# alexandre01/deepsvg

Measured on AMD Instinct MI355X. Metric: SVG icons/sec (train step) hierarchical_ordered d=256, higher is better.
Workload: dtype bf16; 1 GPU; hierarchical_ordered (Hierarchical, use_vae=False) G=8 S=30 d_model=256 ff=512 H=8 L=4x4; full train step = forward + SVGLoss + backward + grad-clip 1.0 + AdamW; dropout 0.1; global_batch=512, batch_per_gpu=512, parallelism=dp1, hip_graph=True, encoder_layout=packed (valid tokens only, exact)

## Files before the change

deepsvg_amd/csrc/dsvg_common.h:

```cpp
#pragma once
#include <hip/hip_runtime.h>
#include <stdint.h>
#include <string.h>
#include <stdio.h>

#define DSVG_F32 0
#define DSVG_BF16 1

typedef uint16_t bf16_t;

extern "C" const char* dsvg_last_error(void);
void dsvg_set_error(const char* fmt, ...);

#define DSVG_CHECK_ARG(cond, ...)                \
    do {                                         \
        if (!(cond)) {                           \
            dsvg_set_error(__VA_ARGS__);         \
            return -1;                           \
        }                                        \
    } while (0)

#define DSVG_LAUNCH_CHECK(name)                                                        \
    do {                                                                               \
        hipError_t _e = hipGetLastError();                                             \
        if (_e != hipSuccess) {                                                        \
            dsvg_set_error("%s: launch failed: %s", name, hipGetErrorString(_e));      \
            return -2;                                                                 \
        }                                                                              \
    } while (0)

#define DSVG_ENSURE_LDS(kern, bytes)                                                                      \
    do {                                                                                                  \
        static size_t _dsvg_cap = 64 * 1024;                                                              \
        if ((size_t)(bytes) > _dsvg_cap) {                                                                \
            (void)hipFuncSetAttribute((const void*)(kern), hipFuncAttributeMaxDynamicSharedMemorySize,    \
                                      (int)(bytes));                                                      \
            _dsvg_cap = (size_t)(bytes);                                                                  \
        }                                                                                                 \
    } while (0)

__device__ __forceinline__ float bf2f(bf16_t h) { return __uint_as_float(((uint32_t)h) << 16); }
typedef __bf16 dsvg_bf2 __attribute__((ext_vector_type(2)));
typedef float dsvg_f2 __attribute__((ext_vector_type(2)));
__device__ __forceinline__ bf16_t f2bf(float f) {
    const __bf16 b = (__bf16)f;
    return __builtin_bit_cast(bf16_t, b);
}
__device__ __forceinline__ uint32_t f2bf_pk(float lo, float hi) {
    const dsvg_f2 v = {lo, hi};
    const dsvg_bf2 b = __builtin_convertvector(v, dsvg_bf2);
    return __builtin_bit_cast(uint32_t, b);
}

template <typename T> struct Elem;
template <> struct Elem<float> {
    typedef float4 raw4;
    static __device__ __forceinline__ float ld(const float* p) { return *p; }
    static __device__ __forceinline__ void st(float* p, float v) { *p = v; }
    static __device__ __forceinline__ void ld4(const float* p, float (&v)[4]) {
        float4 t = *reinterpret_cast<const float4*>(p);
        v[0] = t.x; v[1] = t.y; v[2] = t.z; v[3] = t.w;
    }
    static __device__ __forceinline__ void st4(float* p, const float (&v)[4]) {
        *reinterpret_cast<float4*>(p) = make_float4(v[0], v[1], v[2], v[3]);
    }
};
template <> struct Elem<bf16_t> {
    typedef uint2 raw4;
    static __device__ __forceinline__ float ld(const bf16_t* p) { return bf2f(*p); }
    static __device__ __forceinline__ void st(bf16_t* p, float v) { *p = f2bf(v); }
    static __device__ __forceinline__ void ld4(const bf16_t* p, float (&v)[4]) {
        uint2 t = *reinterpret_cast<const uint2*>(p);
        v[0] = __uint_as_float(t.x << 16); v[1] = __uint_as_float(t.x & 0xffff0000u);
        v[2] = __uint_as_float(t.y << 16); v[3] = __uint_as_float(t.y & 0xffff0000u);
    }
    static __device__ __forceinline__ void st4(bf16_t* p, const float (&v)[4]) {
        uint2 t;
        t.x = f2bf_pk(v[0], v[1]);
        t.y = f2bf_pk(v[2], v[3]);
        *reinterpret_cast<uint2*>(p) = t;
    }
};

__device__ __forceinline__ void row32_load(const float* p, float (&v)[32]) {
#pragma unroll
// ... 42 lines not shown
};
__device__ __forceinline__ DropCtx drop_make(float p, const uint64_t* seed_ptr, uint32_t site) {
    DropCtx c;
    c.on = (p > 0.f) && (seed_ptr != nullptr);
    if (c.on) {
        uint64_t seed = *seed_ptr;
        c.s0 = dsvg_hash32((uint32_t)seed ^ (site * 0x9e3779b1u));
        c.s1 = dsvg_hash32((uint32_t)(seed >> 32) + site * 0x85ebca77u + 0x165667b1u);
        uint32_t t = (uint32_t)(p * 65536.f + 0.5f);
        c.thresh = t > 65535u ? 65535u : t;
        c.scale = 65536.f / (float)(65536u - c.thresh);
    } else {
        c.s0 = c.s1 = 0; c.thresh = 0; c.scale = 1.f;
    }
    return c;
}
__device__ __forceinline__ uint32_t drop_group(const DropCtx& c, uint64_t g) {
    const uint32_t h = dsvg_hash32((uint32_t)g ^ c.s0);
    return (h ^ c.s1) + (uint32_t)(g >> 32) * 0x9e3779b1u;
}
__device__ __forceinline__ uint32_t drop_word(uint32_t h, uint32_t i) {
    const uint32_t c = ((0x7feb352du * (i + 1u)) ^ (0x846ca68bu >> i)) | 1u;
    return (h * c) ^ __umulhi(h, c);
}
__device__ __forceinline__ float drop_mult(const DropCtx& c, uint64_t idx) {
    if (!c.on) return 1.f;
    const uint32_t slot = (uint32_t)idx & 7u;
    const uint32_t w = drop_word(drop_group(c, idx >> 3), slot >> 1);
    const uint32_t draw = (slot & 1u) ? (w >> 16) : (w & 0xffffu);
    return draw < c.thresh ? 0.f : c.scale;
}
__device__ __forceinline__ void drop_mult8(const DropCtx& c, uint64_t idx8, float (&m)[8]) {
    if (!c.on) {
#pragma unroll
        for (int e = 0; e < 8; ++e) m[e] = 1.f;
        return;
    }
    const uint32_t h = drop_group(c, idx8 >> 3);
#pragma unroll
    for (int i = 0; i < 4; ++i) {
        const uint32_t w = drop_word(h, i);
        m[2 * i] = (w & 0xffffu) < c.thresh ? 0.f : c.scale;
        m[2 * i + 1] = (w >> 16) < c.thresh ? 0.f : c.scale;
    }
}

__device__ __forceinline__ uint32_t attn_drop_row(const DropCtx& c, uint64_t row, uint32_t key_block) {
    const uint64_t g = row * 8ull + key_block;
    const uint32_t h = dsvg_hash32((uint32_t)g ^ c.s0);
    return dsvg_hash32(h + (uint32_t)(g >> 32) * 0x9e3779b1u + c.s1);
}
__device__ __forceinline__ float attn_drop_key(const DropCtx& c, uint32_t hrow, uint32_t key) {
    if (!c.on) return 1.f;
    const uint32_t w = drop_word(hrow, (key & 31u) >> 1);
    const uint32_t draw = (key & 1u) ? (w >> 16) : (w & 0xffffu);
    return draw < c.thresh ? 0.f : c.scale;
}
__device__ __forceinline__ float attn_drop_mult(const DropCtx& c, uint64_t row, uint32_t key) {
    if (!c.on) return 1.f;
    return attn_drop_key(c, attn_drop_row(c, row, key >> 5), key);
}

__device__ __forceinline__ float dsvg_gumbel_from_word(uint32_t w) {
    const float u = ((float)(w >> 9) + 0.5f) * (1.f / 8388608.f);
    return -__logf(-__logf(u));
}
__device__ __forceinline__ float dsvg_gumbel(const DropCtx& c, uint64_t row, uint32_t k4, uint32_t col) {
    return dsvg_gumbel_from_word(drop_word(drop_group(c, row * k4 + (col >> 2)), col & 3u));
}

__device__ __forceinline__ float wave_sum(float v) {
#pragma unroll
    for (int o = 32; o > 0; o >>= 1) v += __shfl_xor(v, o, 64);
    return v;
}
__device__ __forceinline__ float wave_max(float v) {
#pragma unroll
    for (int o = 32; o > 0; o >>= 1) v = fmaxf(v, __shfl_xor(v, o, 64));
    return v;
}

static inline int dsvg_cdiv(long long a, long long b) { return (int)((a + b - 1) / b); }

__host__ __device__ inline size_t dsvg_splitk_slice(size_t M, size_t N, bool rowsums) {
    return (M * N + (rowsums ? M : 0) + 3) & ~(size_t)3;
}

int dsvg_reduce_partials_strided(const float* part, int64_t P, int64_t stride, int64_t n, float* out,
                                 int32_t accumulate, hipStream_t st);
int dsvg_reduce_partials_mixed(const float* part, int64_t P, int64_t stride, int64_t n, int64_t n_bf16, float* out,
                               int32_t accumulate, hipStream_t st);
```

deepsvg_amd/csrc/embed.hip:

```cpp
#include "dsvg_common.h"
#include "../../include/dsvg.h"

__global__ void build_masks_kernel(const float* __restrict__ commands, long long n_seq, int S, int G, int eos,
                                   uint64_t* __restrict__ key_mask, int* __restrict__ seq_visible,
                                   uint64_t* __restrict__ group_mask) {
    const long long b = (long long)blockIdx.x * blockDim.x + threadIdx.x;
    if (b >= n_seq) return;
    const float* row = commands + b * S;
    uint64_t km = 0;
    int n_eos = 0;
    bool seen = false;
    for (int s = 0; s < S; ++s) {
        const bool is_eos = ((int)row[s] == eos);
        seen |= is_eos;
        n_eos += is_eos;
        if (!seen) km |= (1ull << s);
    }
    if (key_mask) key_mask[b] = km;
    if (seq_visible) seq_visible[b] = (n_eos < S - 1) ? 1 : 0;
}
__global__ void group_mask_kernel(const int* __restrict__ seq_visible, long long n_icons, int G,
                                  uint64_t* __restrict__ group_mask) {
    const long long n = (long long)blockIdx.x * blockDim.x + threadIdx.x;
    if (n >= n_icons) return;
// ... 173 lines not shown
    hipStream_t st = (hipStream_t)stream;
    hipLaunchKernelGGL(seq_offsets_kernel, dim3(1), dim3(1024), 0, st, key_mask, (long long)n_seq, seq_off);
    DSVG_LAUNCH_CHECK("seq_offsets");
    hipLaunchKernelGGL(pack_tokens_kernel, dim3(dsvg_cdiv(n_seq * S, 256)), dim3(256), 0, st, commands, args, seq_off,
                       (long long)n_seq, S, n_args, packed_commands, packed_args, packed_pos);
    DSVG_LAUNCH_CHECK("pack_tokens");
    return 0;
}

__global__ __launch_bounds__(1024) void seq_offsets_lens_kernel(const int32_t* __restrict__ lens, long long n_seq, int S,
                                                                int32_t* __restrict__ seq_off) {
    __shared__ int part[1024];
    __shared__ int carry;
    if (threadIdx.x == 0) carry = 0;
    __syncthreads();
    for (long long base = 0; base < n_seq; base += 1024) {
        const long long b = base + threadIdx.x;
        const int len = b < n_seq ? min(max(lens[b], 0), S) : 0;
        part[threadIdx.x] = len;
        __syncthreads();
        for (int o = 1; o < 1024; o <<= 1) {
            const int v = threadIdx.x >= o ? part[threadIdx.x - o] : 0;
            __syncthreads();
            part[threadIdx.x] += v;
            __syncthreads();
        }
        if (b < n_seq) seq_off[b] = carry + part[threadIdx.x] - len;
        __syncthreads();
        if (threadIdx.x == 1023) carry += part[1023];
        __syncthreads();
    }
    if (threadIdx.x == 0) seq_off[n_seq] = carry;
}
extern "C" int dsvg_pack_tokens_lens(const float* commands, const float* args, const int32_t* lens, int64_t n_seq,
                                     int32_t S, int32_t n_args, int32_t* seq_off, float* packed_commands,
                                     float* packed_args, int32_t* packed_pos, void* stream) {
    DSVG_CHECK_ARG(commands && args && lens && seq_off && packed_commands && packed_args && packed_pos,
                   "pack_tokens_lens: null pointer");
    DSVG_CHECK_ARG(n_seq > 0 && S > 0 && S <= 256 && n_args > 0 && n_seq * S < (1ll << 31), "pack_tokens_lens: bad shape");
    hipStream_t st = (hipStream_t)stream;
    hipLaunchKernelGGL(seq_offsets_lens_kernel, dim3(1), dim3(1024), 0, st, lens, (long long)n_seq, S, seq_off);
    DSVG_LAUNCH_CHECK("seq_offsets_lens");
    hipLaunchKernelGGL(pack_tokens_kernel, dim3(dsvg_cdiv(n_seq * S, 256)), dim3(256), 0, st, commands, args, seq_off,
                       (long long)n_seq, S, n_args, packed_commands, packed_args, packed_pos);
    DSVG_LAUNCH_CHECK("pack_tokens_lens");
    return 0;
}

template <typename T>
__global__ void embed_gather_kernel(const float* __restrict__ commands, const float* __restrict__ args,
                                    const float* __restrict__ command_embed, const float* __restrict__ arg_embed,
                                    const float* __restrict__ group_embed, const int* __restrict__ groups,
                                    T* __restrict__ A, T* __restrict__ R, long long T_tok, int n_args, int E, int d,
                                    int n_cmd, int n_argvals) {
    const int wa = n_args * E / 4, wr = d / 4;
    const long long total = T_tok * (wa + wr);
    for (long long idx = (long long)blockIdx.x * blockDim.x + threadIdx.x; idx < total;
         idx += (long long)gridDim.x * blockDim.x) {
        const long long t = idx / (wa + wr);
        const int c = (int)(idx % (wa + wr));
        float v[4];
        if (c < wa) {
            const int a = (4 * c) / E, e = (4 * c) % E;
            int iv = (int)args[t * n_args + a] + 1;
            iv = min(max(iv, 0), n_argvals - 1);
            const float4 w = *reinterpret_cast<const float4*>(arg_embed + (size_t)iv * E + e);
            v[0] = w.x; v[1] = w.y; v[2] = w.z; v[3] = w.w;
            Elem<T>::st4(A + t * (long long)(n_args * E) + 4 * c, v);
        } else {
            const int cc = 4 * (c - wa);
            int ic = (int)commands[t];
            ic = min(max(ic, 0), n_cmd - 1);
            float4 w = *reinterpret_cast<const float4*>(command_embed + (size_t)ic * d + cc);
            if (group_embed) {
                const float4 g = *reinterpret_cast<const float4*>(group_embed + (size_t)groups[t] * d + cc);
                w.x += g.x; w.y += g.y; w.z += g.z; w.w += g.w;
            }
            v[0] = w.x; v[1] = w.y; v[2] = w.z; v[3] = w.w;
            Elem<T>::st4(R + t * (long long)d + cc, v);
        }
    }
}

extern "C" int dsvg_embed_gather(int32_t dtype, const float* commands, const float* args, const float* command_embed,
                                 const float* arg_embed, const float* group_embed, const int32_t* groups, void* A,
                                 void* R, int64_t T_tok, int32_t n_args, int32_t E, int32_t d, int32_t n_cmd,
                                 int32_t n_argvals, void* stream) {
    DSVG_CHECK_ARG(commands && args && command_embed && arg_embed && A && R, "embed_gather: null pointer");
    DSVG_CHECK_ARG(T_tok > 0 && (E % 4) == 0 && (d % 4) == 0, "embed_gather: bad shape");
    DSVG_CHECK_ARG(!group_embed || groups, "embed_gather: group_embed needs groups");
    const long long total = T_tok * (long long)(n_args * E / 4 + d / 4);
    const int nb = (int)min((long long)dsvg_cdiv(total, 256), 8192LL);
    hipStream_t st = (hipStream_t)stream;
    if (dtype == DSVG_F32)
        hipLaunchKernelGGL(embed_gather_kernel<float>, dim3(nb), dim3(256), 0, st, commands, args, command_embed,
                           arg_embed, group_embed, groups, (float*)A, (float*)R, (long long)T_tok, n_args, E, d, n_cmd,
                           n_argvals);
    else if (dtype == DSVG_BF16)
        hipLaunchKernelGGL(embed_gather_kernel<bf16_t>, dim3(nb), dim3(256), 0, st, commands, args, command_embed,
                           arg_embed, group_embed, groups, (bf16_t*)A, (bf16_t*)R, (long long)T_tok, n_args, E, d,
                           n_cmd, n_argvals);
    else { dsvg_set_error("embed_gather: bad dtype"); return -1; }
    DSVG_LAUNCH_CHECK("embed_gather");
    return 0;
}

constexpr int ES_TOK_PER_BLOCK = 128;

template <typename T>
__global__ __launch_bounds__(256) void embed_scatter_arg_kernel(const float* __restrict__ args, const T* __restrict__ dA,
                                                                float* __restrict__ part, long long T_tok, int n_args,
                                                                int E, int n_argvals) {
    extern __shared__ float acc[];
    const int tab = n_argvals * E;
    for (int i = threadIdx.x; i < tab; i += 256) acc[i] = 0.f;
    __syncthreads();
    const long long t0 = (long long)blockIdx.x * ES_TOK_PER_BLOCK;
    const long long t1 = min(T_tok, t0 + ES_TOK_PER_BLOCK);
    const int width = n_args * E;
    constexpr int KC = 4, TU = 8;
    int a_of[KC], e_of[KC];
    float acc0[KC] = {0.f, 0.f, 0.f, 0.f};
#pragma unroll
    for (int k = 0; k < KC; ++k) {
        const int c = threadIdx.x + 256 * k;
        a_of[k] = c < width ? c / E : -1;
        e_of[k] = c < width ? c % E : 0;
    }
    for (int c = threadIdx.x + 256 * KC; c < width; c += 256) {
        for (long long t = t0; t < t1; ++t) {
            const float g = Elem<T>::ld(dA + t * width + c);
            int iv = (int)args[t * n_args + c / E] + 1;
            iv = min(max(iv, 0), n_argvals - 1);
            if (g != 0.f) atomicAdd(&acc[iv * E + c % E], g);
        }
    }
    for (long long tb = t0; tb < t1; tb += TU) {
        float g[TU][KC];
        int iv[TU][KC];
#pragma unroll
        for (int u = 0; u < TU; ++u) {
            const long long t = tb + u;
#pragma unroll
            for (int k = 0; k < KC; ++k) {
                const bool ok = t < t1 && a_of[k] >= 0;
                const long long tt = min(t, t1 - 1);
                const float gv = Elem<T>::ld(dA + tt * width + (a_of[k] >= 0 ? threadIdx.x + 256 * k : 0));
                const int av = (int)args[tt * n_args + max(a_of[k], 0)] + 1;
                g[u][k] = ok ? gv : 0.f;
                iv[u][k] = ok ? av : 0;
            }
        }
#pragma unroll
        for (int u = 0; u < TU; ++u)
#pragma unroll
            for (int k = 0; k < KC; ++k) {
                const int row = min(max(iv[u][k], 0), n_argvals - 1);
                if (row == 0) acc0[k] += g[u][k];
                else if (g[u][k] != 0.f) atomicAdd(&acc[row * E + e_of[k]], g[u][k]);
            }
    }
#pragma unroll
    for (int k = 0; k < KC; ++k)
        if (a_of[k] >= 0 && acc0[k] != 0.f) atomicAdd(&acc[e_of[k]], acc0[k]);
    __syncthreads();
    float* dst = part + (size_t)blockIdx.x * tab;
    for (int i = threadIdx.x; i < tab; i += 256) dst[i] = acc[i];
}

typedef __bf16 es_bf16x8 __attribute__((ext_vector_type(8)));
typedef short es_shortx4 __attribute__((ext_vector_type(4)));
typedef float es_floatx16 __attribute__((ext_vector_type(16)));
constexpr int ESM_LD = 11 * 64 + 8;
__device__ __forceinline__ int es_rowmap(int r, int h2) { return (r & 3) + 8 * (r >> 2) + 4 * h2; }
__global__ __launch_bounds__(512) void embed_scatter_arg_mfma_kernel(const float* __restrict__ args,
                                                                     const bf16_t* __restrict__ dA, float* __restrict__ part,
// ... 44 lines not shown
#pragma unroll
                    for (int e = 0; e < 4; ++e)
                        w[e] = (tok_idx[2 * e] == v ? 0x3f80u : 0u) | (tok_idx[2 * e + 1] == v ? 0x3f800000u : 0u);
                    union { es_bf16x8 v8; uint4 u; } f;
                    f.u = make_uint4(w[0], w[1], w[2], w[3]);
                    oh[vt][ks] = f.v8;
                }
            }
#pragma unroll
            for (int ntile = 0; ntile < 2; ++ntile) {
                const int col0 = a * 64 + 32 * ntile;
#pragma unroll
                for (int ks = 0; ks < 2; ++ks) {
                    const int g = lane >> 4, q16 = lane & 15;
                    const int row = 16 * ks + 4 * (g >> 1) + (q16 >> 2);
                    const int col = col0 + 16 * (g & 1) + 4 * (q16 & 3);
                    union { es_bf16x8 v8; es_shortx4 h[2]; } fa;
                    fa.h[0] = __builtin_amdgcn_ds_read_tr16_b64_v4i16(
                        (es_shortx4 __attribute__((address_space(3)))*)(&img[row * ESM_LD + col]));
                    fa.h[1] = __builtin_amdgcn_ds_read_tr16_b64_v4i16(
                        (es_shortx4 __attribute__((address_space(3)))*)(&img[(row + 8) * ESM_LD + col]));
                    acc[0][ntile] = __builtin_amdgcn_mfma_f32_32x32x16_bf16(fa.v8, oh[0][ks], acc[0][ntile], 0, 0, 0);
                    if (n_vt == 2)
                        acc[1][ntile] = __builtin_amdgcn_mfma_f32_32x32x16_bf16(fa.v8, oh[1][ks], acc[1][ntile], 0, 0, 0);
                }
            }
        }
        __syncthreads();
    }
    float* dst = part + (size_t)blockIdx.x * n_argvals * 64;
#pragma unroll
    for (int vt = 0; vt < 2; ++vt) {
        if (vt >= n_vt) break;
        const int v = (vt == 0 ? 32 * wave : 256) + li;
        if (v >= n_argvals) continue;
#pragma unroll
        for (int ntile = 0; ntile < 2; ++ntile)
#pragma unroll
            for (int r = 0; r < 16; ++r) dst[(size_t)v * 64 + 32 * ntile + es_rowmap(r, h2)] = acc[vt][ntile][r];
    }
}

template <typename T>
__global__ __launch_bounds__(256) void embed_scatter_row_kernel(const float* __restrict__ commands,
                                                                const int* __restrict__ groups,
                                                                const T* __restrict__ dR, float* __restrict__ part_cmd,
                                                                float* __restrict__ part_grp, long long T_tok, int d,
                                                                int n_cmd, int n_groups, int g_lo, int g_win) {
    extern __shared__ float acc[];
    float* acc_c = acc;
    float* acc_g = acc + n_cmd * d;
    const bool do_cmd = g_lo == 0;
    for (int i = threadIdx.x; i < (n_cmd + g_win) * d; i += 256) acc[i] = 0.f;
    __syncthreads();
    const long long t0 = (long long)blockIdx.x * ES_TOK_PER_BLOCK;
    const long long t1 = min(T_tok, t0 + ES_TOK_PER_BLOCK);
    constexpr int TU = 8;
    for (int c = threadIdx.x; c < d; c += 256) {
        for (long long tb = t0; tb < t1; tb += TU) {
            float g[TU];
            int ic[TU], ig[TU];
#pragma unroll
            for (int u = 0; u < TU; ++u) {
                const long long t = min(tb + u, t1 - 1);
                g[u] = Elem<T>::ld(dR + t * d + c);
                ic[u] = (int)commands[t];
                ig[u] = part_grp ? groups[t] - g_lo : -1;
            }
#pragma unroll
            for (int u = 0; u < TU; ++u) {
                if (tb + u < t1 && g[u] != 0.f) {
                    if (do_cmd) acc_c[min(max(ic[u], 0), n_cmd - 1) * d + c] += g[u];
                    if (ig[u] >= 0 && ig[u] < g_win) acc_g[ig[u] * d + c] += g[u];
                }
            }
        }
    }
    __syncthreads();
    if (do_cmd)
        for (int i = threadIdx.x; i < n_cmd * d; i += 256) part_cmd[(size_t)blockIdx.x * n_cmd * d + i] = acc_c[i];
    if (part_grp)
        for (int i = threadIdx.x; i < g_win * d; i += 256)
            part_grp[(size_t)blockIdx.x * n_groups * d + (size_t)g_lo * d + i] = acc_g[i];
}

extern "C" int64_t dsvg_embed_scatter_workspace_bytes(int64_t T_tok, int32_t n_args, int32_t E, int32_t d,
                                                      int32_t n_cmd, int32_t n_argvals, int32_t n_groups) {
    const int64_t nb = dsvg_cdiv(T_tok, ES_TOK_PER_BLOCK);
    return nb * ((int64_t)n_argvals * E + (int64_t)(n_cmd + n_groups) * d) * (int64_t)sizeof(float);
}

extern "C" int dsvg_embed_scatter(int32_t dtype, const float* commands, const float* args, const int32_t* groups,
                                  const void* dA, const void* dR, float* d_arg_embed, float* d_command_embed,
                                  float* d_group_embed, int64_t T_tok, int32_t n_args, int32_t E, int32_t d,
                                  int32_t n_cmd, int32_t n_argvals, int32_t n_groups, float* workspace,
                                  int64_t workspace_bytes, void* stream) {
    DSVG_CHECK_ARG(commands && args && dA && dR && d_arg_embed && d_command_embed, "embed_scatter: null pointer");
    DSVG_CHECK_ARG(!d_group_embed || (groups && n_groups > 0), "embed_scatter: group table needs groups");
    if (!d_group_embed) n_groups = 0;
    DSVG_CHECK_ARG(workspace && workspace_bytes >= dsvg_embed_scatter_workspace_bytes(T_tok, n_args, E, d, n_cmd,
                                                                                     n_argvals, n_groups),
                   "embed_scatter: workspace too small");
    hipStream_t st = (hipStream_t)stream;
    const int nb = dsvg_cdiv(T_tok, ES_TOK_PER_BLOCK);
    const int tab = n_argvals * E;
    float* part_arg = workspace;
    float* part_cmd = part_arg + (size_t)nb * tab;
    float* part_grp = n_groups ? part_cmd + (size_t)nb * n_cmd * d : nullptr;
    const size_t lds_a = (size_t)tab * sizeof(float);
    int g_cap = (int)((128 * 1024) / ((size_t)d * sizeof(float))) - n_cmd;
    DSVG_CHECK_ARG(lds_a <= 160 * 1024 && g_cap >= 1, "embed_scatter: tables too large for LDS");
    const int g_win0 = n_groups < g_cap ? n_groups : g_cap;
    const size_t lds_r = (size_t)(n_cmd + g_win0) * d * sizeof(float);
    if (dtype == DSVG_F32) {
        auto ka = embed_scatter_arg_kernel<float>;
        auto kr = embed_scatter_row_kernel<float>;
        DSVG_ENSURE_LDS(ka, lds_a);
        DSVG_ENSURE_LDS(kr, lds_r);
        hipLaunchKernelGGL(ka, dim3(nb), dim3(256), lds_a, st, args, (const float*)dA, part_arg, (long long)T_tok, n_args, E, n_argvals);
        for (int g_lo = 0; g_lo == 0 || g_lo < n_groups; g_lo += g_cap) {
            const int win = n_groups - g_lo < g_cap ? n_groups - g_lo : g_cap;
            hipLaunchKernelGGL(kr, dim3(nb), dim3(256), lds_r, st, commands, groups, (const float*)dR, part_cmd, part_grp,
                               (long long)T_tok, d, n_cmd, n_groups, g_lo, win > 0 ? win : 0);
        }
    } else if (dtype == DSVG_BF16) {
        auto ka = embed_scatter_arg_kernel<bf16_t>;
        auto kr = embed_scatter_row_kernel<bf16_t>;
        DSVG_ENSURE_LDS(ka, lds_a);
        DSVG_ENSURE_LDS(kr, lds_r);
        static const bool mfma_off = getenv("DSVG_EMBED_SCATTER_MFMA") && atoi(getenv("DSVG_EMBED_SCATTER_MFMA")) == 0;
        if (!mfma_off && E == 64 && n_args == 11 && n_argvals > 224 && n_argvals <= 288 && ((uintptr_t)dA & 15) == 0) {
            const size_t lds_m = (size_t)32 * ESM_LD * 2 + 32 * 16 * sizeof(int);
            DSVG_ENSURE_LDS(embed_scatter_arg_mfma_kernel, lds_m);
            hipLaunchKernelGGL(embed_scatter_arg_mfma_kernel, dim3(nb), dim3(512), lds_m, st, args, (const bf16_t*)dA, part_arg,
                               (long long)T_tok, n_args, n_argvals);
        } else
        hipLaunchKernelGGL(ka, dim3(nb), dim3(256), lds_a, st, args, (const bf16_t*)dA, part_arg, (long long)T_tok, n_args, E, n_argvals);
        for (int g_lo = 0; g_lo == 0 || g_lo < n_groups; g_lo += g_cap) {
            const int win = n_groups - g_lo < g_cap ? n_groups - g_lo : g_cap;
            hipLaunchKernelGGL(kr, dim3(nb), dim3(256), lds_r, st, commands, groups, (const bf16_t*)dR, part_cmd, part_grp,
                               (long long)T_tok, d, n_cmd, n_groups, g_lo, win > 0 ? win : 0);
        }
    } else { dsvg_set_error("embed_scatter: bad dtype"); return -1; }
    DSVG_LAUNCH_CHECK("embed_scatter");
    int rc = dsvg_reduce_partials_strided(part_arg, nb, tab, tab, d_arg_embed, 0, st);
    if (rc) return rc;
    rc = dsvg_reduce_partials_strided(part_cmd, nb, (int64_t)n_cmd * d, (int64_t)n_cmd * d, d_command_embed, 0, st);
    if (rc) return rc;
    if (n_groups) rc = dsvg_reduce_partials_strided(part_grp, nb, (int64_t)n_groups * d, (int64_t)n_groups * d, d_group_embed, 0, st);
    return rc;
}

template <typename T>
__global__ void add_pos_fwd_kernel(const T* __restrict__ x, const float* __restrict__ pos, T* __restrict__ y,
                                   long long n_tok, int S, int d, float drop_p, uint32_t site, const uint64_t* seed) {
    const DropCtx dc = drop_make(drop_p, seed, site);
    if ((d & 7) == 0) {
        const int vpr8 = d / 8;
        const long long total8 = n_tok * vpr8;
        for (long long idx = (long long)blockIdx.x * blockDim.x + threadIdx.x; idx < total8;
             idx += (long long)gridDim.x * blockDim.x) {
            const long long t = idx / vpr8;
            const int c = 8 * (int)(idx % vpr8);
            const int s = (int)(t % S);
            float a[4] = {0.f, 0.f, 0.f, 0.f}, b[4] = {0.f, 0.f, 0.f, 0.f}, m[8];
            if (x) { Elem<T>::ld4(x + t * d + c, a); Elem<T>::ld4(x + t * d + c + 4, b); }
            const float4 p0 = *reinterpret_cast<const float4*>(pos + (size_t)s * d + c);
            const float4 p1 = *reinterpret_cast<const float4*>(pos + (size_t)s * d + c + 4);
            drop_mult8(dc, (uint64_t)t * d + c, m);
            a[0] = (a[0] + p0.x) * m[0]; a[1] = (a[1] + p0.y) * m[1]; a[2] = (a[2] + p0.z) * m[2]; a[3] = (a[3] + p0.w) * m[3];
            b[0] = (b[0] + p1.x) * m[4]; b[1] = (b[1] + p1.y) * m[5]; b[2] = (b[2] + p1.z) * m[6]; b[3] = (b[3] + p1.w) * m[7];
            Elem<T>::st4(y + t * d + c, a);
            Elem<T>::st4(y + t * d + c + 4, b);
        }
        return;
    }
    const int vpr = d / 4;
    const long long total = n_tok * vpr;
    for (long long idx = (long long)blockIdx.x * blockDim.x + threadIdx.x; idx < total;
         idx += (long long)gridDim.x * blockDim.x) {
        const long long t = idx / vpr;
        const int c = 4 * (int)(idx % vpr);
        const int s = (int)(t % S);
        float v[4] = {0.f, 0.f, 0.f, 0.f};
        if (x) Elem<T>::ld4(x + t * d + c, v);
        const float4 pe = *reinterpret_cast<const float4*>(pos + (size_t)s * d + c);
        const uint64_t e = (uint64_t)t * d + c;
        v[0] = (v[0] + pe.x) * drop_mult(dc, e);
        v[1] = (v[1] + pe.y) * drop_mult(dc, e + 1);
        v[2] = (v[2] + pe.z) * drop_mult(dc, e + 2);
        v[3] = (v[3] + pe.w) * drop_mult(dc, e + 3);
        Elem<T>::st4(y + t * d + c, v);
    }
}

template <typename T>
__global__ void drop_copy_kernel(const T* __restrict__ dy, T* __restrict__ dx, long long n4, float drop_p,
                                 uint32_t site, const uint64_t* seed) {
    const DropCtx dc = drop_make(drop_p, seed, site);
    for (long long i = (long long)blockIdx.x * blockDim.x + threadIdx.x; i < n4; i += (long long)gridDim.x * blockDim.x) {
        float v[4];
        Elem<T>::ld4(dy + 4 * i, v);
#pragma unroll
        for (int e = 0; e < 4; ++e) v[e] *= drop_mult(dc, (uint64_t)(4 * i + e));
        Elem<T>::st4(dx + 4 * i, v);
    }
}

template <typename T>
__global__ void drop_apply8_kernel(const T* __restrict__ x, T* __restrict__ y, long long n8, float drop_p,
                                   uint32_t site, const uint64_t* seed) {
    const DropCtx dc = drop_make(drop_p, seed, site);
    for (long long i = (long long)blockIdx.x * blockDim.x + threadIdx.x; i < n8; i += (long long)gridDim.x * blockDim.x) {
        float a[4], b[4], m[8];
        Elem<T>::ld4(x + 8 * i, a);
        Elem<T>::ld4(x + 8 * i + 4, b);
        drop_mult8(dc, (uint64_t)(8 * i), m);
#pragma unroll
        for (int e = 0; e < 4; ++e) { a[e] *= m[e]; b[e] *= m[4 + e]; }
        Elem<T>::st4(y + 8 * i, a);
// ... 378 lines not shown
```

deepsvg_amd/csrc/gemm.hip:

```cpp
#include "dsvg_common.h"
#include "../../include/dsvg.h"
#include "gemm_common.h"
int dsvg_gemm_group_flush(hipStream_t st);
#include <map>
#include <mutex>
#include <vector>

template <typename T>
__global__ void gemm_naive_kernel(dsvg_gemm_desc p, int k_begin, int k_end, float* part, float* rs) {
    long long idx = (long long)blockIdx.x * blockDim.x + threadIdx.x;
    if (idx >= (long long)p.M * p.N) return;
    int m = (int)(idx / p.N), n = (int)(idx % p.N);
    const T* A = (const T*)p.A;
    const T* B = (const T*)p.B;
    DropCtx adc = drop_make(p.a_drop_p, p.seed, p.a_drop_site);
    float acc = 0.f, asum = 0.f;
    for (int k = k_begin; k < k_end; ++k) {
        float a, b;
        if (p.a_kc) {
            a = Elem<T>::ld(A + (size_t)m * p.lda + k);
            a *= drop_mult(adc, (uint64_t)m * p.a_drop_ld + k);
        } else {
            a = Elem<T>::ld(A + (size_t)k * p.lda + m);
            a *= drop_mult(adc, (uint64_t)k * p.a_drop_ld + m);
// ... 584 lines not shown
    if (n_bf16 > 0) { if (wide) DSVG_RP(4, 64, true); else DSVG_RP(4, 16, true); }
    else if (vec) { if (wide) DSVG_RP(4, 64, false); else DSVG_RP(4, 16, false); }
    else if (narrow) DSVG_RP(1, 4, false);
    else     { if (wide) DSVG_RP(1, 64, false); else DSVG_RP(1, 16, false); }
#undef DSVG_RP
    DSVG_LAUNCH_CHECK("reduce_partials");
    return 0;
}

constexpr int CS_ROWS_MIN = 16, CS_ROWS_MAX = 1024;
template <typename T>
__global__ __launch_bounds__(256) void colsum_kernel(const T* __restrict__ A, long long lda, long long M, int N,
                                                     float* __restrict__ part, float drop_p, uint32_t site,
                                                     const uint64_t* seed, int cpb, int vec_ok, int rows_per_block) {
    constexpr int VEC = 16 / (int)sizeof(T);
    __shared__ float red[256][VEC + 1];
    const DropCtx dc = drop_make(drop_p, seed, site);
    const int cl = threadIdx.x % cpb, rg = threadIdx.x / cpb, nrg = 256 / cpb;
    const int c0 = (blockIdx.y * cpb + cl) * VEC;
    const long long r0 = (long long)blockIdx.x * rows_per_block;
    const long long r1 = min(M, r0 + rows_per_block);
    float acc[VEC];
#pragma unroll
    for (int e = 0; e < VEC; ++e) acc[e] = 0.f;
    if (c0 < N) {
        if (vec_ok && c0 + VEC <= N) {
            for (long long r = r0 + rg; r < r1; r += nrg) {
                float v[VEC];
                if (VEC == 4) {
                    float t[4];
                    Elem<T>::ld4(A + r * lda + c0, t);
#pragma unroll
                    for (int e = 0; e < 4; ++e) v[e % VEC] = t[e];
                } else {
                    float t0[4], t1[4];
                    Elem<T>::ld4(A + r * lda + c0, t0);
                    Elem<T>::ld4(A + r * lda + c0 + 4, t1);
#pragma unroll
                    for (int e = 0; e < 4; ++e) { v[e] = t0[e]; v[(e + 4) % VEC] = t1[e]; }
                }
                if (VEC == 8 && dc.on && !(N & 7)) {
                    float m8[8];
                    drop_mult8(dc, (uint64_t)r * N + c0, m8);
#pragma unroll
                    for (int e = 0; e < VEC; ++e) acc[e] += v[e] * m8[e % 8];
                } else {
#pragma unroll
                    for (int e = 0; e < VEC; ++e) acc[e] += v[e] * drop_mult(dc, (uint64_t)r * N + c0 + e);
                }
            }
        } else {
            for (long long r = r0 + rg; r < r1; r += nrg)
#pragma unroll
                for (int e = 0; e < VEC; ++e)
                    if (c0 + e < N) acc[e] += Elem<T>::ld(A + r * lda + c0 + e) * drop_mult(dc, (uint64_t)r * N + c0 + e);
        }
    }
#pragma unroll
    for (int e = 0; e < VEC; ++e) red[threadIdx.x][e] = acc[e];
    __syncthreads();
    if (rg == 0 && c0 < N) {
#pragma unroll
        for (int e = 0; e < VEC; ++e) {
            if (c0 + e < N) {
                float s = 0.f;
                for (int g = 0; g < nrg; ++g) s += red[g * cpb + cl][e];
                part[(long long)blockIdx.x * N + c0 + e] = s;
            }
        }
    }
}

extern "C" int64_t dsvg_gemm_workspace_bytes(int32_t M, int32_t N, int32_t split_k) {
    if (split_k <= 1) return 0;
    return (int64_t)split_k * (int64_t)dsvg_splitk_slice(M, N, true) * (int64_t)sizeof(float);
}

extern "C" int dsvg_reduce_partials(const float* partial, int64_t P, int64_t n, float* out,
                                    int32_t accumulate, void* stream) {
    DSVG_CHECK_ARG(partial && out && P >= 0 && n >= 0, "reduce_partials: bad args");
    return dsvg_reduce_partials_strided(partial, P, n, n, out, accumulate, (hipStream_t)stream);
}

extern "C" int64_t dsvg_colsum_workspace_bytes(int64_t M, int32_t N) {
    return (int64_t)dsvg_cdiv(M, CS_ROWS_MIN) * N * (int64_t)sizeof(float);
}

extern "C" int dsvg_colsum(int32_t dtype, const void* A, int64_t lda, int64_t M, int32_t N, float* out,
                           int32_t accumulate, float drop_p, uint32_t drop_site, const uint64_t* seed,
                           float* workspace, int64_t workspace_bytes, void* stream) {
    DSVG_CHECK_ARG(A && out && M > 0 && N > 0, "colsum: bad args");
    DSVG_CHECK_ARG(workspace && workspace_bytes >= dsvg_colsum_workspace_bytes(M, N),
                   "colsum: workspace too small (%lld < %lld)", (long long)workspace_bytes,
                   (long long)dsvg_colsum_workspace_bytes(M, N));
    hipStream_t st = (hipStream_t)stream;
    DSVG_CHECK_ARG(dtype == DSVG_F32 || dtype == DSVG_BF16, "colsum: bad dtype %d", dtype);
    const int vec = dtype == DSVG_F32 ? 4 : 8;
    const int chunks = dsvg_cdiv(N, vec);
    int cpb = 8;
    while (cpb < 64 && cpb < chunks) cpb *= 2;
    const int vec_ok = !(lda % vec) && !((uintptr_t)A & 15);
    const int col_blocks = dsvg_cdiv(chunks, cpb);
    long long rpb = M / max(1, 1024 / col_blocks);
    rpb = rpb < CS_ROWS_MIN ? CS_ROWS_MIN : (rpb > CS_ROWS_MAX ? CS_ROWS_MAX : rpb);
    const int nb = dsvg_cdiv(M, rpb);
    dim3 grid(nb, col_blocks);
    if (dtype == DSVG_F32)
        hipLaunchKernelGGL(colsum_kernel<float>, grid, dim3(256), 0, st, (const float*)A, (long long)lda,
                           (long long)M, N, workspace, drop_p, drop_site, seed, cpb, vec_ok, (int)rpb);
    else
        hipLaunchKernelGGL(colsum_kernel<bf16_t>, grid, dim3(256), 0, st, (const bf16_t*)A, (long long)lda,
                           (long long)M, N, workspace, drop_p, drop_site, seed, cpb, vec_ok, (int)rpb);
    DSVG_LAUNCH_CHECK("colsum");
    return dsvg_reduce_partials(workspace, nb, N, out, accumulate, stream);
}

int dsvg_gemm_bf16_launch(const dsvg_gemm_desc& d, int k_chunk, int nsplit, float* part, float* rs_part,
                          hipStream_t st, int* part_is_bf16);

extern "C" int dsvg_gemm(const dsvg_gemm_desc* dp, void* stream) {
    DSVG_CHECK_ARG(dp, "gemm: null desc");
    dsvg_gemm_desc d = *dp;
    hipStream_t st = (hipStream_t)stream;
    DSVG_CHECK_ARG(d.dtype == DSVG_F32 || d.dtype == DSVG_BF16, "gemm: bad dtype %d", d.dtype);
    DSVG_CHECK_ARG(d.M > 0 && d.N > 0 && d.K > 0, "gemm: bad shape %d %d %d", d.M, d.N, d.K);
    DSVG_CHECK_ARG(d.A && d.B && d.C, "gemm: null operand");
    DSVG_CHECK_ARG((d.drop_p <= 0.f && d.a_drop_p <= 0.f) || d.seed, "gemm: dropout needs a seed pointer");
    if (d.dtype == DSVG_F32) d.c_f32 = 1;
    const int split = d.split_k > 1 ? d.split_k : 1;
    float* part = nullptr;
    int k_chunk = d.K;
    if (split > 1) {
        DSVG_CHECK_ARG(d.c_f32, "gemm: split_k needs fp32 output");
        DSVG_CHECK_ARG(!d.bias && !d.res && !d.gate && d.act == 0 && d.drop_p <= 0.f,
                       "gemm: split_k does not support an epilogue");
        DSVG_CHECK_ARG(d.workspace && d.workspace_bytes >= dsvg_gemm_workspace_bytes(d.M, d.N, split),
                       "gemm: split_k workspace too small");
        DSVG_CHECK_ARG(d.ldc == d.N, "gemm: split_k needs a dense C (ldc == N)");
        part = d.workspace;
        k_chunk = ((d.K + split - 1) / split + 63) / 64 * 64;
    }
    int nsplit = (d.K + k_chunk - 1) / k_chunk;
    if (split > 1 && (split % 8) == 0) nsplit = split;
    DSVG_CHECK_ARG(!d.rowsum || part, "gemm: rowsum needs split_k > 1");
    float* rs_part = d.rowsum ? part + (size_t)d.M * d.N : nullptr;
    const size_t slice = dsvg_splitk_slice(d.M, d.N, d.rowsum != nullptr);

    int part_bf16 = 0;
    bool use_naive = d.impl == 1;
    if (d.dtype == DSVG_F32) {
        if ((d.lda & 3) || (d.ldb & 3) || ((uintptr_t)d.A & 15) || ((uintptr_t)d.B & 15)) use_naive = true;
    } else {
        const int Kp = (d.K + 7) / 8 * 8;
        if ((d.lda & 7) || (d.ldb & 7) || ((uintptr_t)d.A & 15) || ((uintptr_t)d.B & 15)) use_naive = true;
        if ((d.a_kc && d.lda < Kp) || (d.b_kc && d.ldb < Kp)) use_naive = true;
        if (!d.a_kc && d.lda < ((d.M + 7) / 8) * 8) use_naive = true;
        if (!d.b_kc && d.ldb < ((d.N + 7) / 8) * 8) use_naive = true;
    }
    if (use_naive) {
        const long long total = (long long)d.M * d.N;
        for (int z = 0; z < nsplit; ++z) {
            const int kb = z * k_chunk, ke = min(d.K, kb + k_chunk);
            float* pz = part ? part + (size_t)z * slice : nullptr;
            float* rz = rs_part ? rs_part + (size_t)z * slice : nullptr;
            if (d.dtype == DSVG_F32)
                hipLaunchKernelGGL(gemm_naive_kernel<float>, dim3(dsvg_cdiv(total, 256)), dim3(256), 0, st, d, kb, ke, pz, rz);
            else
                hipLaunchKernelGGL(gemm_naive_kernel<bf16_t>, dim3(dsvg_cdiv(total, 256)), dim3(256), 0, st, d, kb, ke, pz, rz);
        }
        DSVG_LAUNCH_CHECK("gemm_naive");
    } else if (d.dtype == DSVG_F32) {
        const int tiles_m = dsvg_cdiv(d.M, BM), tiles_n = dsvg_cdiv(d.N, BN);
        const int nwg = tiles_m * tiles_n;
        dim3 grid(nwg, nsplit);
        if (nsplit > 1 && (nsplit % 8) == 0) grid = dim3(nwg * nsplit, 1);
#define DSVG_F32V(AK, BK)                                                                                              \
    do {                                                                                                               \
        if (rs_part) hipLaunchKernelGGL((gemm_f32_mfma_kernel<AK, BK, true>), grid, dim3(256), 0, st, d, tiles_n, nwg, \
                                        k_chunk, part, rs_part);                                                       \
        else hipLaunchKernelGGL((gemm_f32_mfma_kernel<AK, BK, false>), grid, dim3(256), 0, st, d, tiles_n, nwg,        \
                                k_chunk, part, rs_part);                                                               \
    } while (0)
        if (d.a_kc && d.b_kc) DSVG_F32V(true, true);
        else if (d.a_kc && !d.b_kc) DSVG_F32V(true, false);
        else if (!d.a_kc && d.b_kc) DSVG_F32V(false, true);
        else DSVG_F32V(false, false);
#undef DSVG_F32V
        DSVG_LAUNCH_CHECK("gemm_f32_mfma");
    } else {
// ... 23 lines not shown
```

Before: 92530 icons/s.

## Add vectorized bf16 embed gather and register-accumulating embed scatter kernels

Adds a bf16 embed-gather kernel that first stages per-token indices in shared memory, then writes 8-element packed bf16 vectors. Adds a row-scatter kernel that stages a token tile of dR in LDS and accumulates command and group gradients in per-thread register vectors, replacing the windowed LDS-accumulator launches. Both are on by default behind env knobs. It also computes the colsum workspace size from the real grid rather than the minimum rows per block. Dynamic indexing into the register vectors may spill to scratch, and the gains are limited to small embedding kernels.

```diff
diff --git a/deepsvg_amd/csrc/dsvg_common.h b/deepsvg_amd/csrc/dsvg_common.h
--- a/deepsvg_amd/csrc/dsvg_common.h
+++ b/deepsvg_amd/csrc/dsvg_common.h
@@ -1,6 +1,7 @@
 #pragma once
 #include <hip/hip_runtime.h>
 #include <stdint.h>
+#include <stdlib.h>
 #include <string.h>
 #include <stdio.h>
 
@@ -209,6 +210,11 @@
 
 static inline int dsvg_cdiv(long long a, long long b) { return (int)((a + b - 1) / b); }
 
+static inline bool dsvg_knob_on(const char* name) {
+    const char* v = getenv(name);
+    return !(v && atoi(v) == 0);
+}
+
 __host__ __device__ inline size_t dsvg_splitk_slice(size_t M, size_t N, bool rowsums) {
     return (M * N + (rowsums ? M : 0) + 3) & ~(size_t)3;
 }
diff --git a/deepsvg_amd/csrc/embed.hip b/deepsvg_amd/csrc/embed.hip
--- a/deepsvg_amd/csrc/embed.hip
+++ b/deepsvg_amd/csrc/embed.hip
@@ -279,6 +279,66 @@
     }
 }
 
+constexpr int EG_TOK = 32;
+__device__ __forceinline__ uint4 eg_pack8(const float4 lo, const float4 hi) {
+    return make_uint4(f2bf_pk(lo.x, lo.y), f2bf_pk(lo.z, lo.w), f2bf_pk(hi.x, hi.y), f2bf_pk(hi.z, hi.w));
+}
+__global__ __launch_bounds__(256) void embed_gather16_kernel(const float* __restrict__ commands, const float* __restrict__ args,
+                                                             const float* __restrict__ command_embed,
+                                                             const float* __restrict__ arg_embed,
+                                                             const float* __restrict__ group_embed,
+                                                             const int* __restrict__ groups, bf16_t* __restrict__ A,
+                                                             bf16_t* __restrict__ R, long long T_tok, int n_args, int E, int d,
+                                                             int n_cmd, int n_argvals) {
+    extern __shared__ int eg_rows[];
+    const int ni = n_args + 2;
+    const long long t0 = (long long)blockIdx.x * EG_TOK;
+    const int nt = (int)min((long long)EG_TOK, T_tok - t0);
+    for (int i = threadIdx.x; i < nt * ni; i += 256) {
+        const int tl = i / ni, a = i - tl * ni;
+        const long long t = t0 + tl;
+        const void* p = a < n_args ? (const void*)(args + t * n_args + a)
+                                   : (a > n_args && group_embed) ? (const void*)(groups + t) : (const void*)(commands + t);
+        const uint32_t raw = *reinterpret_cast<const uint32_t*>(p);
+        const int fi = (int)__uint_as_float(raw);
+        eg_rows[i] = a < n_args ? min(max(fi + 1, 0), n_argvals - 1)
+                                : a == n_args ? min(max(fi, 0), n_cmd - 1) : (group_embed ? (int)raw : 0);
+    }
+    __syncthreads();
+    const int epa = E / 8, wa = n_args * epa, wr = d / 8;
+    uint4* Ab = reinterpret_cast<uint4*>(A + t0 * (long long)(n_args * E));
+    const int total_a = nt * wa;
+#pragma unroll 4
+    for (int i = threadIdx.x; i < total_a; i += 256) {
+        const int sa = i / epa, e = 8 * (i - sa * epa);
+        const int tl = sa / n_args, a = sa - tl * n_args;
+        const float* src = arg_embed + (size_t)eg_rows[tl * ni + a] * E + e;
+        Ab[i] = eg_pack8(reinterpret_cast<const float4*>(src)[0], reinterpret_cast<const float4*>(src)[1]);
+    }
+    uint4* Rb = reinterpret_cast<uint4*>(R + t0 * (long long)d);
+    const int total_r = nt * wr;
+    if (group_embed) {
+#pragma unroll 4
+        for (int i = threadIdx.x; i < total_r; i += 256) {
+            const int tl = i / wr, cc = 8 * (i - tl * wr);
+            const float* src = command_embed + (size_t)eg_rows[tl * ni + n_args] * d + cc;
+            const float* gsr = group_embed + (size_t)eg_rows[tl * ni + n_args + 1] * d + cc;
+            float4 lo = reinterpret_cast<const float4*>(src)[0], hi = reinterpret_cast<const float4*>(src)[1];
+            const float4 gl = reinterpret_cast<const float4*>(gsr)[0], gh = reinterpret_cast<const float4*>(gsr)[1];
+            lo.x += gl.x; lo.y += gl.y; lo.z += gl.z; lo.w += gl.w;
+            hi.x += gh.x; hi.y += gh.y; hi.z += gh.z; hi.w += gh.w;
+            Rb[i] = eg_pack8(lo, hi);
+        }
+    } else {
+#pragma unroll 4
+        for (int i = threadIdx.x; i < total_r; i += 256) {
+            const int tl = i / wr, cc = 8 * (i - tl * wr);
+            const float* src = command_embed + (size_t)eg_rows[tl * ni + n_args] * d + cc;
+            Rb[i] = eg_pack8(reinterpret_cast<const float4*>(src)[0], reinterpret_cast<const float4*>(src)[1]);
+        }
+    }
+}
+
 extern "C" int dsvg_embed_gather(int32_t dtype, const float* commands, const float* args, const float* command_embed,
                                  const float* arg_embed, const float* group_embed, const int32_t* groups, void* A,
                                  void* R, int64_t T_tok, int32_t n_args, int32_t E, int32_t d, int32_t n_cmd,
@@ -289,6 +349,15 @@
     const long long total = T_tok * (long long)(n_args * E / 4 + d / 4);
     const int nb = (int)min((long long)dsvg_cdiv(total, 256), 8192LL);
     hipStream_t st = (hipStream_t)stream;
+    if (dtype == DSVG_BF16 && dsvg_knob_on("DSVG_EMBED_GATHER16") && n_args > 0 && (E % 8) == 0 && (d % 8) == 0 &&
+        (((uintptr_t)A | (uintptr_t)R | (uintptr_t)command_embed | (uintptr_t)arg_embed | (uintptr_t)group_embed) & 15) == 0 &&
+        T_tok < (1ll << 31) * EG_TOK) {
+        hipLaunchKernelGGL(embed_gather16_kernel, dim3(dsvg_cdiv(T_tok, EG_TOK)), dim3(256),
+                           (size_t)EG_TOK * (n_args + 2) * sizeof(int), st, commands, args, command_embed, arg_embed,
+                           group_embed, groups, (bf16_t*)A, (bf16_t*)R, (long long)T_tok, n_args, E, d, n_cmd, n_argvals);
+        DSVG_LAUNCH_CHECK("embed_gather");
+        return 0;
+    }
     if (dtype == DSVG_F32)
         hipLaunchKernelGGL(embed_gather_kernel<float>, dim3(nb), dim3(256), 0, st, commands, args, command_embed,
                            arg_embed, group_embed, groups, (float*)A, (float*)R, (long long)T_tok, n_args, E, d, n_cmd,
@@ -499,6 +568,76 @@
     if (part_grp)
         for (int i = threadIdx.x; i < g_win * d; i += 256)
             part_grp[(size_t)blockIdx.x * n_groups * d + (size_t)g_lo * d + i] = acc_g[i];
+}
+
+constexpr int ESR_ROWS = 8, ESR_GROWS = 32, ESR_STAGE = 16;
+constexpr int ESR_TU = 8;
+typedef float es_f16v __attribute__((ext_vector_type(16)));
+typedef float es_f32v __attribute__((ext_vector_type(32)));
+__global__ __launch_bounds__(256) void embed_scatter_row_reg_kernel(const float* __restrict__ commands,
+                                                                    const int* __restrict__ groups,
+                                                                    const bf16_t* __restrict__ dR,
+                                                                    float* __restrict__ part_cmd, float* __restrict__ part_grp,
+                                                                    long long T_tok, int d, int n_cmd, int n_groups) {
+    extern __shared__ __attribute__((aligned(16))) unsigned char esr_smem[];
+    bf16_t* tile = reinterpret_cast<bf16_t*>(esr_smem);
+    int* trow = reinterpret_cast<int*>(esr_smem + (size_t)ESR_STAGE * 256 * 16);
+    const long long t0 = (long long)blockIdx.x * ES_TOK_PER_BLOCK;
+    const int nt = (int)min((long long)ES_TOK_PER_BLOCK, T_tok - t0);
+    const int total = nt * (d / 8);
+    const uint4* src = reinterpret_cast<const uint4*>(dR + t0 * d);
+    uint4 v[ESR_STAGE];
+#pragma unroll
+    for (int k = 0; k < ESR_STAGE; ++k) v[k] = src[min((int)threadIdx.x + 256 * k, total - 1)];
+    {
+        const int tl = min((int)threadIdx.x, nt - 1);
+        const int ic = min(max((int)commands[t0 + tl], 0), n_cmd - 1);
+        const int* gp = part_grp ? groups : reinterpret_cast<const int*>(commands);
+        const int igl = gp[t0 + tl];
+        const int ig = part_grp ? igl : -1;
+        trow[threadIdx.x] = ic | ((ig >= 0 && ig < n_groups ? ig : 255) << 8);
+    }
+#pragma unroll
+    for (int k = 0; k < ESR_STAGE; ++k) reinterpret_cast<uint4*>(tile)[threadIdx.x + 256 * k] = v[k];
+    __syncthreads();
+    for (int c = threadIdx.x; c < d; c += 256) {
+        es_f16v ac;
+        es_f32v ag;
+#pragma unroll
+        for (int k = 0; k < 16; ++k) ac[k] = 0.f;
+#pragma unroll
+        for (int k = 0; k < ESR_GROWS; ++k) ag[k] = 0.f;
+        for (int tb = 0; tb < nt; tb += ESR_TU) {
+            float g[ESR_TU];
+            int rw[ESR_TU];
+#pragma unroll
+            for (int u = 0; u < ESR_TU; ++u) {
+                const int tl = min(tb + u, nt - 1);
+                g[u] = bf2f(tile[tl * d + c]);
+                rw[u] = trow[tl];
+            }
+#pragma unroll
+            for (int u = 0; u < ESR_TU; ++u) {
+                if (tb + u < nt) {
+                    const float gv = g[u];
+                    const int r = __builtin_amdgcn_readfirstlane(rw[u]);
+                    const int ic = r & 255, ig = r >> 8;
+                    const float a0 = ac[ic];
+                    ac[ic] = gv != 0.f ? a0 + gv : a0;
+                    if (ig < ESR_GROWS) {
+                        const float a1 = ag[ig];
+                        ag[ig] = gv != 0.f ? a1 + gv : a1;
+                    }
+                }
+            }
+        }
+#pragma unroll
+        for (int k = 0; k < ESR_ROWS; ++k)
+            if (k < n_cmd) part_cmd[(size_t)blockIdx.x * n_cmd * d + (size_t)k * d + c] = ac[k];
+#pragma unroll
+        for (int k = 0; k < ESR_GROWS; ++k)
+            if (k < n_groups) part_grp[(size_t)blockIdx.x * n_groups * d + (size_t)k * d + c] = ag[k];
+    }
 }
 
 extern "C" int64_t dsvg_embed_scatter_workspace_bytes(int64_t T_tok, int32_t n_args, int32_t E, int32_t d,
@@ -553,6 +692,13 @@
                                (long long)T_tok, n_args, n_argvals);
         } else
         hipLaunchKernelGGL(ka, dim3(nb), dim3(256), lds_a, st, args, (const bf16_t*)dA, part_arg, (long long)T_tok, n_args, E, n_argvals);
+        if (dsvg_knob_on("DSVG_EMBED_SCATTER_ROW_REG") && (d % 8) == 0 && d <= 256 && n_cmd <= ESR_ROWS &&
+            n_groups <= ESR_GROWS && ((uintptr_t)dR & 15) == 0) {
+            const size_t lds_t = (size_t)ESR_STAGE * 256 * 16 + 256 * sizeof(int);
+            DSVG_ENSURE_LDS(embed_scatter_row_reg_kernel, lds_t);
+            hipLaunchKernelGGL(embed_scatter_row_reg_kernel, dim3(nb), dim3(256), lds_t, st, commands, groups,
+                               (const bf16_t*)dR, part_cmd, part_grp, (long long)T_tok, d, n_cmd, n_groups);
+        } else
         for (int g_lo = 0; g_lo == 0 || g_lo < n_groups; g_lo += g_cap) {
             const int win = n_groups - g_lo < g_cap ? n_groups - g_lo : g_cap;
             hipLaunchKernelGGL(kr, dim3(nb), dim3(256), lds_r, st, commands, groups, (const bf16_t*)dR, part_cmd, part_grp,
diff --git a/deepsvg_amd/csrc/gemm.hip b/deepsvg_amd/csrc/gemm.hip
--- a/deepsvg_amd/csrc/gemm.hip
+++ b/deepsvg_amd/csrc/gemm.hip
@@ -690,8 +690,23 @@
     return dsvg_reduce_partials_strided(partial, P, n, n, out, accumulate, (hipStream_t)stream);
 }
 
+struct ColsumGrid { int cpb, col_blocks, nb; long long rpb; };
+static ColsumGrid colsum_grid(int vec, int64_t M, int32_t N) {
+    ColsumGrid g;
+    const int chunks = dsvg_cdiv(N, vec);
+    g.cpb = 8;
+    while (g.cpb < 64 && g.cpb < chunks) g.cpb *= 2;
+    g.col_blocks = dsvg_cdiv(chunks, g.cpb);
+    long long rpb = M / max(1, 1024 / g.col_blocks);
+    g.rpb = rpb < CS_ROWS_MIN ? CS_ROWS_MIN : (rpb > CS_ROWS_MAX ? CS_ROWS_MAX : rpb);
+    g.nb = dsvg_cdiv(M, g.rpb);
+    return g;
+}
+
 extern "C" int64_t dsvg_colsum_workspace_bytes(int64_t M, int32_t N) {
-    return (int64_t)dsvg_cdiv(M, CS_ROWS_MIN) * N * (int64_t)sizeof(float);
+    if (M <= 0 || N <= 0) return 0;
+    const int nb4 = colsum_grid(4, M, N).nb, nb8 = colsum_grid(8, M, N).nb;
+    return (int64_t)(nb4 > nb8 ? nb4 : nb8) * N * (int64_t)sizeof(float);
 }
 
 extern "C" int dsvg_colsum(int32_t dtype, const void* A, int64_t lda, int64_t M, int32_t N, float* out,
@@ -704,15 +719,11 @@
     hipStream_t st = (hipStream_t)stream;
     DSVG_CHECK_ARG(dtype == DSVG_F32 || dtype == DSVG_BF16, "colsum: bad dtype %d", dtype);
     const int vec = dtype == DSVG_F32 ? 4 : 8;
-    const int chunks = dsvg_cdiv(N, vec);
-    int cpb = 8;
-    while (cpb < 64 && cpb < chunks) cpb *= 2;
     const int vec_ok = !(lda % vec) && !((uintptr_t)A & 15);
-    const int col_blocks = dsvg_cdiv(chunks, cpb);
-    long long rpb = M / max(1, 1024 / col_blocks);
-    rpb = rpb < CS_ROWS_MIN ? CS_ROWS_MIN : (rpb > CS_ROWS_MAX ? CS_ROWS_MAX : rpb);
-    const int nb = dsvg_cdiv(M, rpb);
-    dim3 grid(nb, col_blocks);
+    const ColsumGrid cg = colsum_grid(vec, M, N);
+    const int cpb = cg.cpb, nb = cg.nb;
+    const long long rpb = cg.rpb;
+    dim3 grid(nb, cg.col_blocks);
     if (dtype == DSVG_F32)
         hipLaunchKernelGGL(colsum_kernel<float>, grid, dim3(256), 0, st, (const float*)A, (long long)lda,
                            (long long)M, N, workspace, drop_p, drop_site, seed, cpb, vec_ok, (int)rpb);
```

Result: no change. 93240 icons/s (median of 6 runs) (+0.8%).
